# resemble-ai/chatterbox

Hardware: AMD Instinct MI355X
Metric: audio-sec/wall-sec (xRT) + p50 first-audio latency, Multilingual-V3 500M (higher is better)
Workload: dtype f32 (T3: exact fp32 MFMA; S3Gen: every fp32 operand = 2 fp16 planes h + l/2048 = 22 significand bits, 3 fp16 MFMA products per fp32 product in two fp32 accumulators: error at or below the exact-fp32 MFMA path; operand range checked on the device, bf16x6 repeat otherwise)

## Files before the change

### chatterbox_amd/_lib.py

```python
import ctypes
import os

import torch

_HERE = os.path.dirname(os.path.abspath(__file__))
LIB_PATH = os.environ.get("CBX_LIB_PATH") or os.path.join(_HERE, "libcbx_hip.so")

c_f = ctypes.c_void_p
c_int, c_long, c_float = ctypes.c_int, ctypes.c_long, ctypes.c_float


ABI_VERSION = 16


class GemmParams(ctypes.Structure):
    _fields_ = [
        ("A", c_f), ("W", c_f), ("C", c_f), ("bias", c_f), ("R", c_f), ("C2", c_f),
        ("act1_param", c_f), ("act2_param", c_f), ("lens", c_f),
        ("M", c_int), ("N", c_int), ("K", c_int),
        ("Cin", c_int), ("taps", c_int), ("dil", c_int), ("stride", c_int), ("pad_left", c_int), ("up", c_int),
        ("Tin", c_int), ("nz1", c_int), ("nz2", c_int), ("w_kn", c_int), ("swiglu", c_int),
        ("act1", c_int), ("act2", c_int),
        ("act1_slope", c_float), ("act2_slope", c_float), ("alpha", c_float), ("beta", c_float),
        ("lda", c_long), ("a_s1", c_long), ("a_s2", c_long),
# ... 118 lines not shown


class PrefillEmbed(ctypes.Structure):
    _fields_ = ([(k, c_int) for k in ("B", "cfg", "n_bos", "abs_pos", "S", "pos0", "dim")] + [("bos_id", ctypes.c_longlong), ("meta", c_f), ("ids", c_f), ("cond", c_f),
                                                                                               ("cond_stride", c_long)]
                + [(k, c_f) for k in ("text_emb", "text_pos", "speech_emb", "speech_pos", "x", "positions", "cache_rows", "last")])


class PlanesRef(ctypes.Structure):
    _fields_ = [("p", c_f), ("ld", c_long), ("lo", c_long)]


class CfmTBlock(ctypes.Structure):
    _fields_ = [(k, c_f) for k in ("n1_w", "n1_b", "n3_w", "n3_b", "bo", "b1", "b2")] + [(k, PlanesRef) for k in ("wqkv", "wo", "w1", "w2")]


class CfmStage(ctypes.Structure):
    _fields_ = ([(k, PlanesRef) for k in ("c1", "c2", "res", "tail")]
                + [(k, c_f) for k in ("c1_b", "n1_w", "n1_b", "c2_b", "n2_w", "n2_b", "res_b", "tail_b")]
                + [("cin", c_int), ("n_tb", c_int), ("tb", ctypes.POINTER(CfmTBlock))])


class CfmSolve(ctypes.Structure):
    _fields_ = ([(k, c_int) for k in ("n_stages", "rows", "B", "n_steps", "cfg", "fused_qkv", "fused_ln")]
                + [("T", c_long), ("cfg_rate", c_float), ("dt", ctypes.POINTER(c_float)), ("stages", ctypes.POINTER(CfmStage)),
                   ("fin_c", PlanesRef), ("fin_proj", PlanesRef)]
                + [(k, c_f) for k in ("fin_c_b", "fin_n_w", "fin_n_b", "fin_proj_b", "tbias", "lens", "xin")]
                + [("xinP", PlanesRef)] + [(k, c_f) for k in ("ra", "rb", "x", "v")]
                + [(k, PlanesRef) for k in ("aP", "hP", "qkP", "attP", "ffP", "xP", "yP", "catP", "vtP")]
                + [("gemm_tile", c_int), ("attn_version", c_int)])


class Conformer(ctypes.Structure):
    _fields_ = [(k, c_f) for k in ("ln_mha_w", "ln_mha_b", "w4", "b4", "wpos", "wo", "bo", "ln_ff_w", "ln_ff_b", "w1", "b1", "w2", "b2")]


class S3Encode(ctypes.Structure):
    _fields_ = ([(k, c_int) for k in ("B", "N", "n_enc", "n_up", "precision")] + [(k, c_f) for k in ("ids", "lens", "lens2")]
                + [(k, c_f) for k in ("emb", "e_w", "e_b", "e_lnw", "e_lnb", "u_w", "u_b", "u_lnw", "u_lnb", "pl1_w", "pl1_b", "pl2_w", "pl2_b", "up_w", "up_b",
                                      "after_w", "after_b", "proj_w", "proj_b")]
                + [("enc", ctypes.POINTER(Conformer)), ("up_enc", ctypes.POINTER(Conformer)), ("pe", c_f), ("pe2", c_f)]
                + [(k, c_f) for k in ("x0", "xa", "y1", "x2", "xu", "xb", "h", "q4", "pp", "att", "ff", "mu")])


class HiftF0(ctypes.Structure):
    _fields_ = [("B", c_int), ("T", c_long), ("mel", c_f), ("lens", c_f), ("f0_w", c_f * 5), ("f0_b", c_f * 5), ("cls_w", c_f), ("cls_b", c_f), ("src_w", c_f),
                ("src_b", c_float), ("phase", c_f), ("noise", c_f), ("buf0", c_f), ("buf1", c_f), ("f0", c_f), ("s", c_f), ("cum", c_f)]
# ... 112 lines not shown
    "cbx_hift_istft_rows_f32": ([c_f, c_f, c_f, c_int, c_long, c_long, c_float, c_int, c_f], c_int),
}


class CbxError(RuntimeError):
    pass


def _load():
    if not os.path.exists(LIB_PATH):
        raise ImportError(
            f"{LIB_PATH} is missing: build it with `python -m chatterbox_amd.build` (hipcc --offload-arch=gfx950). "
            "chatterbox_amd has no CPU / eager fallback.")
    lib = ctypes.CDLL(LIB_PATH)
    for name, (args, res) in _SIGS.items():
        try:
            fn = getattr(lib, name)
        except AttributeError as e:
            raise ImportError(f"libcbx_hip.so does not export {name} (stale build?)") from e
        fn.argtypes = args
        fn.restype = res
    if lib.cbx_abi_version() != ABI_VERSION:
        raise ImportError("libcbx_hip.so ABI version mismatch")
    return lib


lib = _load()


def check(rc, what=""):
    if rc != 0:
        raise CbxError(f"{what}: rc={rc}: {lib.cbx_last_error().decode(errors='replace')}")
```

### chatterbox_amd/csrc/attention_planes.hip

```cpp
#include <stdlib.h>
#include "cbx_common.h"

namespace {

typedef _Float16 f16x4 __attribute__((ext_vector_type(4)));
typedef _Float16 f16x8 __attribute__((ext_vector_type(8)));
typedef unsigned u32x4 __attribute__((ext_vector_type(4)));

__device__ __attribute__((aligned(16))) const unsigned cbx_attn_zero_page[4] = {0u, 0u, 0u, 0u};
typedef const __attribute__((address_space(1))) void* gptr_t;
typedef __attribute__((address_space(3))) void* lptr_t;

struct FlashPlArgs {
    const _Float16* q; const _Float16* k; const _Float16* vt; _Float16* o; const int* key_lens;
    int Tq, Tk;
    long q_sb, q_st, q_lo, k_sb, k_st, k_lo, vt_sb, vt_sd, vt_lo, o_sb, o_st, o_lo;
    float scale;
    int causal;
    int diag;
};

constexpr int PKT = 64;
constexpr int PL_TILE = 64 * 8 * 16;
constexpr int PL_STAGE = 4 * PL_TILE;
// ... 435 lines not shown
    const float l_tot = l_run + half_swap(l_run);
    const float inv = l_tot > 0.f ? 1.0f / l_tot : 0.f;
    if (qi < a.Tq) {
        _Float16* op = a.o + (long)z * a.o_sb + (long)qi * a.o_st + head * 64;
#pragma unroll
        for (int d = 0; d < 2; ++d)
#pragma unroll
            for (int g = 0; g < 4; ++g) {
                unsigned h0, l0, h1, l1;
                cbx_split2(ot[d][g * 4 + 0] * inv, ot[d][g * 4 + 1] * inv, h0, l0);
                cbx_split2(ot[d][g * 4 + 2] * inv, ot[d][g * 4 + 3] * inv, h1, l1);
                *reinterpret_cast<uint2*>(op + d * 32 + 8 * g + 4 * lh) = make_uint2(h0, h1);
                *reinterpret_cast<uint2*>(op + a.o_lo + d * 32 + 8 * g + 4 * lh) = make_uint2(l0, l1);
            }
    }
}

}

static int g_attn_pl_version = 0;
extern "C" int cbx_set_attn_planes_version(int v) {
    g_attn_pl_version = v;
    return 0;
}

extern "C" int cbx_flash_attn_planes_v(const void* q, const void* k, const void* vt, void* o, const int* key_lens, int nz1, int n_heads, int Tq,
                                       int Tk, long q_sb, long q_st, long q_lo, long k_sb, long k_st, long k_lo, long vt_sb, long vt_sd,
                                       long vt_lo, long o_sb, long o_st, long o_lo, float scale, int causal, int version, void* stream) {
    CBX_REQUIRE(version >= 0 && version <= 6, "flash_attn_planes: version %d (0 = default, 1 .. 6)", version);
    CBX_REQUIRE(q && k && vt && o, "flash_attn_planes: null operand");
    CBX_REQUIRE(Tq > 0 && Tk > 0 && nz1 > 0 && n_heads > 0, "flash_attn_planes: bad shape");
    CBX_REQUIRE((q_sb | q_st | q_lo | k_sb | k_st | k_lo | vt_sb | vt_sd | vt_lo) % 8 == 0 &&
                    (((uintptr_t)q | (uintptr_t)k | (uintptr_t)vt) & 15) == 0,
                "flash_attn_planes: q / k / v^T planes must be 16-byte aligned (strides and plane offsets multiples of 8 halves)");
    CBX_REQUIRE((o_sb | o_st | o_lo) % 4 == 0 && ((uintptr_t)o & 7) == 0, "flash_attn_planes: output planes must be 8-byte aligned");
    CBX_REQUIRE(vt_sd >= (Tk + 7) / 8 * 8, "flash_attn_planes: a V^T row must hold Tk rounded up to 8 keys (got stride %ld for Tk = %d)", vt_sd, Tk);
    FlashPlArgs a{reinterpret_cast<const _Float16*>(q), reinterpret_cast<const _Float16*>(k), reinterpret_cast<const _Float16*>(vt),
                  reinterpret_cast<_Float16*>(o), key_lens, Tq, Tk, q_sb, q_st, q_lo, k_sb, k_st, k_lo, vt_sb, vt_sd, vt_lo, o_sb, o_st, o_lo,
                  scale, causal, 0};
#ifdef CBX_DIAG
    a.diag = getenv("CBX_ATTN_DIAG") ? atoi(getenv("CBX_ATTN_DIAG")) : 0;
#endif
    const int forced = version ? version : g_attn_pl_version;
    const bool short_seq = forced == 0 && Tk <= 768 && (long)((Tq + 255) / 256) * n_heads * nz1 > 128;
    const int ver = forced ? forced : short_seq ? 1 : 4;
    const bool v2ok = !causal && k_st >= k_lo + 64 && (long)Tk * k_st * 2 < 0x7fffffffL && 64 * vt_sd * 2 < 0x7fffffffL && vt_sd >= vt_lo;
    if (ver >= 2 && v2ok) {
        constexpr int lds = 3 * PL_STAGE;
        static unsigned long long configured = 0;
        const int dev = cbx_device();
        if (!(configured >> dev & 1)) {
            hipError_t e1 = hipFuncSetAttribute(reinterpret_cast<const void*>(flash_attn_pl2_kernel<true>), hipFuncAttributeMaxDynamicSharedMemorySize, lds);
            hipError_t e2 = hipFuncSetAttribute(reinterpret_cast<const void*>(flash_attn_pl2_kernel<false>), hipFuncAttributeMaxDynamicSharedMemorySize, lds);
            hipError_t e3 = hipFuncSetAttribute(reinterpret_cast<const void*>((flash_attn_pl2_kernel<false, true>)), hipFuncAttributeMaxDynamicSharedMemorySize, lds);
            hipError_t e4 = hipFuncSetAttribute(reinterpret_cast<const void*>((flash_attn_pl2_kernel<false, true, 4>)), hipFuncAttributeMaxDynamicSharedMemorySize, lds);
            hipError_t e5 = hipFuncSetAttribute(reinterpret_cast<const void*>((flash_attn_pl2_kernel<false, true, 8, true>)), hipFuncAttributeMaxDynamicSharedMemorySize, lds);
            if (e4 == hipSuccess) e4 = e5;
            if (e3 == hipSuccess) e3 = e4;
            if (e2 == hipSuccess) e2 = e3;
            if (e1 != hipSuccess || e2 != hipSuccess) return cbx_set_error((int)(e1 != hipSuccess ? e1 : e2), "flash_attn_planes: cannot reserve %d B of LDS", lds);
            configured |= 1ull << dev;
        }
        dim3 grid2((Tq + 255) / 256, n_heads, nz1);
        const bool small_grid = forced == 0 && (long)grid2.x * n_heads * nz1 <= 128;
        if (ver == 5 || small_grid) hipLaunchKernelGGL((flash_attn_pl2_kernel<false, true, 4>), dim3((Tq + 127) / 128, n_heads, nz1), dim3(256), lds, (hipStream_t)stream, a);
        else if (ver == 6) hipLaunchKernelGGL((flash_attn_pl2_kernel<false, true, 8, true>), grid2, dim3(512), lds, (hipStream_t)stream, a);
        else if (ver == 3) hipLaunchKernelGGL(flash_attn_pl2_kernel<true>, grid2, dim3(512), lds, (hipStream_t)stream, a);
// ... 16 lines not shown
```

### chatterbox_amd/csrc/cbx_common.h

```cpp
#pragma once
#include <hip/hip_runtime.h>
#include <stdint.h>
#include <stdio.h>
#include "../../include/cbx.h"

typedef float f32x4 __attribute__((ext_vector_type(4)));
typedef float f32x16 __attribute__((ext_vector_type(16)));

#ifndef CBX_WT
#define CBX_WT 1
#endif
__device__ __forceinline__ void cbx_store_out(float* p, float v) {
#if CBX_WT == 1
    asm volatile("global_store_dword %0, %1, off sc1" ::"v"(p), "v"(v) : "memory");
#elif CBX_WT == 2
    asm volatile("global_store_dword %0, %1, off sc0 sc1" ::"v"(p), "v"(v) : "memory");
#elif CBX_WT == 3
    __builtin_nontemporal_store(v, p);
#else
    *p = v;
#endif
}
__device__ __forceinline__ void cbx_store_out4(float* p, f32x4 v) {
#if CBX_WT == 1
    asm volatile("global_store_dwordx4 %0, %1, off sc1\n\ts_nop 1" ::"v"(p), "v"(v) : "memory");
#elif CBX_WT == 2
    asm volatile("global_store_dwordx4 %0, %1, off sc0 sc1\n\ts_nop 1" ::"v"(p), "v"(v) : "memory");
#elif CBX_WT == 3
    __builtin_nontemporal_store(v, reinterpret_cast<f32x4*>(p));
#else
    *reinterpret_cast<f32x4*>(p) = v;
#endif
}
#define CBX_F16_LO_SCALE 2048.0f
int* cbx_range_flag();
int cbx_wave_frame_ms(const char* who, const float* wav, const long* row_off, const int* row_len, int R, long nf, double* ws, void* stream);
#ifdef __HIPCC__
__device__ __forceinline__ void cbx_amax4(float& amax, const f32x4 v) {
    asm("v_max3_f32 %0, |%1|, |%2|, %0" : "+v"(amax) : "v"(v[0]), "v"(v[1]));
    asm("v_max3_f32 %0, |%1|, |%2|, %0" : "+v"(amax) : "v"(v[2]), "v"(v[3]));
}
__device__ __forceinline__ void cbx_split2(float v0, float v1, unsigned& h, unsigned& l) {
    typedef _Float16 cbx_h2 __attribute__((ext_vector_type(2)));
    typedef float cbx_f2 __attribute__((ext_vector_type(2)));
    const cbx_f2 v = {v0, v1};
    h = __builtin_bit_cast(unsigned, __builtin_convertvector(v, cbx_h2));
    const cbx_f2 t = v * CBX_F16_LO_SCALE;
    asm("v_fma_mixlo_f16 %0, %1, %2, %3 op_sel:[0,0,0] op_sel_hi:[1,0,0]" : "=v"(l) : "v"(h), "s"(-CBX_F16_LO_SCALE), "v"(t[0]));
    asm("v_fma_mixhi_f16 %0, %1, %2, %3 op_sel:[1,0,0] op_sel_hi:[1,0,0]\n\ts_nop 1" : "+v"(l) : "v"(h), "s"(-CBX_F16_LO_SCALE), "v"(t[1]));
}
#endif

static inline int cbx_device() {
    int d = 0;
    return (hipGetDevice(&d) == hipSuccess && d >= 0 && d < 64) ? d : 0;
}

int cbx_stream_coresident(hipStream_t st);
// ... 274 lines not shown
```

### chatterbox_amd/csrc/stage_seams.hip

```cpp
#include "cbx_common.h"

namespace {

inline cbx_planes_t cols(const cbx_planes_t& P, long c0) { return cbx_planes_t{(char*)P.p + 2 * c0, P.ld, P.lo}; }
inline cbx_planes_t rows_from(const cbx_planes_t& P, long r0) { return cbx_planes_t{(char*)P.p + 2 * r0 * P.ld, P.ld, P.lo}; }

struct CfmCtx {
    const cbx_cfm_t* d;
    void* stream;
    int rows;
    long T, M;

    int conv(const cbx_planes_t& src, const cbx_planes_t& w, int N, int cin, int taps, float* out, const cbx_planes_t* outp, const float* bias,
             const float* R) const {
        cbx_gemm_pl_t g{};
        g.A = src.p, g.W = w.p, g.C = out, g.P = outp ? outp->p : nullptr, g.bias = bias, g.R = R;
        g.M = (int)T, g.N = N, g.K = taps * cin, g.Cin = cin, g.taps = taps, g.dil = 1, g.stride = 1, g.pad_left = taps - 1, g.Tin = (int)T, g.nz1 = rows;
        g.act = CBX_ACT_NONE, g.act_slope = 0.0f, g.alpha = 1.0f;
        g.lda = src.ld, g.a_lo = src.lo, g.a_s1 = T * src.ld;
        g.ldw = w.ld, g.w_lo = w.lo;
        if (out) g.ldc = N, g.c_s1 = T * N;
        if (R) g.ldr = N, g.r_s1 = T * N;
        if (outp) g.ldp = outp->ld, g.p_lo = outp->lo, g.p_s1 = T * outp->ld;
        g.tile = d->gemm_tile;
// ... 74 lines not shown
        return rc;
    }

    int estimator(const float* tbias) const {
        const int n = d->n_stages, n_mid = n - 2;
        const cbx_planes_t skip = cols(d->catP, 256), xh = d->catP;
        int rc;
        if ((rc = block(0, d->xinP, skip, tbias))) return rc;
        cbx_planes_t cur = n_mid == 0 ? xh : d->yP;
        if ((rc = conv(skip, d->stages[0].tail, 256, 256, 3, nullptr, &cur, d->stages[0].tail_b, nullptr))) return rc;
        for (int k = 1; k <= n_mid; ++k) {
            const cbx_planes_t nxt = k == n_mid ? xh : d->xP;
            if ((rc = block(k, cur, nxt, tbias))) return rc;
            cur = nxt;
        }
        if ((rc = block(n - 1, d->catP, d->xP, tbias))) return rc;
        if ((rc = conv(d->xP, d->stages[n - 1].tail, 256, 256, 3, nullptr, &d->yP, d->stages[n - 1].tail_b, nullptr))) return rc;
        if ((rc = conv(d->yP, d->fin_c, 256, 256, 3, d->ra, nullptr, d->fin_c_b, nullptr))) return rc;
        if ((rc = ln_planes(d->ra, d->aP, d->fin_n_w, d->fin_n_b, nullptr, CBX_ACT_MISH))) return rc;
        return conv(d->aP, d->fin_proj, 80, 256, 1, d->v, nullptr, d->fin_proj_b, nullptr);
    }
};

}

extern "C" int cbx_cfm_solve(const cbx_cfm_t* d, void* stream) {
    CBX_REQUIRE(d && d->stages && d->n_stages >= 2 && d->dt && d->tbias && d->xin && d->v && d->ra && d->rb && d->x, "cfm_solve: null descriptor field");
    CBX_REQUIRE(d->B >= 1 && d->T >= 1 && d->n_steps >= 1 && d->rows == (d->cfg ? 2 * d->B : d->B), "cfm_solve: rows must be B (no CFG) or 2 B (CFG)");
    CBX_REQUIRE(d->T % 2 == 0 && (long)d->rows * d->T > 32 && ((long)d->rows * d->T + 512) * 4096 < (1L << 31),
                "cfm_solve: the plane-format path needs an even T, rows * T > 32 and 31-bit operand offsets (rows * T = %ld)", (long)d->rows * d->T);
    for (int k = 0; k < d->n_stages; ++k) {
        const cbx_cfm_stage_t& s = d->stages[k];
        CBX_REQUIRE(s.n_tb >= 1 && s.tb && s.cin % 32 == 0, "cfm_solve: stage %d needs transformer blocks and cin %% 32 == 0", k);
        CBX_REQUIRE((s.tail.p != nullptr) == (k == 0 || k == d->n_stages - 1), "cfm_solve: the down and the up stage (only) end in a conv");
    }
    CfmCtx c{d, stream, d->rows, d->T, (long)d->rows * d->T};
    for (int k = 0; k < d->n_steps; ++k) {
        int rc;
        if (k && (rc = cbx_split_planes_f32(d->xin, d->xinP.p, c.M, 80, 320, d->xinP.ld, d->xinP.lo, stream))) return rc;
        if ((rc = c.estimator(d->tbias + (long)k * d->n_stages * 256))) return rc;
        if ((rc = cbx_cfm_euler_f32(d->xin, d->v, d->B, d->T, 80, 320, 80, d->T * 320, d->T * 80, d->dt[k], d->cfg_rate, d->cfg, stream))) return rc;
    }
    return 0;
}

namespace {

struct HiftCtx {
    const cbx_hift_t* d;
    void* stream;

    struct Conv {
        const float *x, *w, *bias, *res = nullptr, *p1 = nullptr, *p2 = nullptr;
        float *out, *out2 = nullptr;
        const int* lens = nullptr;
        long Tin, Tout, ldx, xs, ldo, os;
        int N, taps, cin, dil = 1, stride = 1, pad_left = 0, act1 = CBX_ACT_NONE, act2 = CBX_ACT_NONE;
        float slope1 = 0.0f, slope2 = 0.0f, alpha = 1.0f, beta = 0.0f;
    };
    int run(const Conv& c) const {
        cbx_gemm_t g{};
        g.A = c.x, g.W = c.w, g.C = c.out, g.bias = c.bias, g.R = c.res, g.C2 = c.out2, g.act1_param = c.p1, g.act2_param = c.p2, g.lens = c.lens;
        g.M = (int)c.Tout, g.N = c.N, g.K = c.taps * c.cin, g.Cin = c.cin, g.taps = c.taps, g.dil = c.dil, g.stride = c.stride, g.pad_left = c.pad_left;
        g.up = 1, g.Tin = (int)c.Tin, g.nz1 = d->B, g.nz2 = 1;
        g.act1 = c.act1, g.act2 = c.act2, g.act1_slope = c.slope1, g.act2_slope = c.slope2, g.alpha = c.alpha, g.beta = c.beta;
        g.lda = c.ldx, g.a_s1 = c.xs, g.ldw = (long)c.taps * c.cin, g.ldc = c.ldo, g.c_s1 = c.os;
        if (c.res) g.ldr = c.ldo, g.r_s1 = c.os;
// ... 195 lines not shown
```

### chatterbox_amd/engine.py

```python
import contextlib
import math
import os
import time
import warnings
from dataclasses import dataclass
from typing import Optional

import torch

from . import ops
from .hift import HiFTEngine
from .s3gen import FlowEngine
from .t3 import T3Engine, START_SPEECH, STOP_SPEECH

SPEECH_VOCAB = 6561
SAMPLES_PER_TOKEN = 960


RANGE_TRIPS = 0


def _range_checked(eng, run, check=True):
    out = run()
    if check and 16 in (eng.flow.precision, eng.hift.precision) and ops.range_flag_tripped():
# ... 439 lines not shown
        if d.join is not None:
            wavs = _joined_on_host(wavs.get("formatted", wavs["out"]), wavs["rec"], wavs["n"], d.fmt, wavs.get("pauses"), self._truncated(toks))
        self.last_timing["total_s"] = time.perf_counter() - t0
        return (wavs, st) if alignment is None else (wavs, st, alignment)

    @staticmethod
    def _truncated(toks):
        return [not bool((t == STOP_SPEECH).any()) for t in toks]
    @torch.inference_mode()
    def synthesize_pipelined(self, jobs, co_resident=True, host_threads=True, t3_in_flight=2, stream_priorities=(-1, 0), t3_pair=None, **kw):
        import threading
        jobs = [_checked_job(job) for job in jobs]
        for job in jobs:
            if "guard" in job:
                job["guard"] = self.t3.check_guard(job["guard"])
                if kw.get("ban_eos") or kw.get("ban_from", 0) > 0:
                    raise ValueError(GUARD_BANS)
        torch.cuda.set_device(self.dev)
        self._pipeline_streams(stream_priorities)
        t3_kw = {k: kw[k] for k in ("max_new_tokens", "temperature", "top_p", "min_p", "repetition_penalty", "cfg_weight", "ban_eos",
                                    "ban_from") if k in kw}
        job_kw = lambda job: dict(t3_kw, **{k: job[k] for k in ("temperature", "top_p", "min_p", "repetition_penalty", "cfg_weight", "guard") if k in job})
        self.co_resident(bool(co_resident))
        from ._lib import check, lib
        attr = bool(co_resident) and t3_in_flight < 2
        check(lib.cbx_set_stream_coresident(self._s_voc.cuda_stream, int(attr)), "cbx_set_stream_coresident")
        torch.cuda.synchronize()

        def enqueue_t3(job, box):
            try:
                torch.cuda.set_device(self.dev)
                with torch.inference_mode(), torch.cuda.stream(self._s_t3):
                    box["handle"] = self.t3.generate(job["t3_conds"], job["text_tokens"], async_mode=True, uniforms=job.get("uniforms"), seeds=job.get("seeds"), **job_kw(job))
            except BaseException as e:
                box["error"] = e

        def vocode_job(job, st):
            wavs, _ = self.vocode(st, job["gen_ref"], z=job.get("z"), phase=job.get("phase"), noise=job.get("noise"), generator=job.get("generator"), seeds=job.get("seeds"),
                                  speed=job.get("speed"), n_cfm_timesteps=kw.get("n_cfm_timesteps", 10), drop_last_token=kw.get("drop_last_token", True), sync=False,
                                  **({k: job[k] for k in ("join", "format", "loudness", "pauses", "pitch", "warp", "true_peak") if k in job}))
            if "warp" in job:
                job["_fit"] = self.last_fit
            return wavs

        def to_host(job, wavs, pinned):
            copy = (lambda w: torch.empty(w.shape, dtype=w.dtype, pin_memory=True).copy_(w, non_blocking=True)) if pinned else (lambda w: w.cpu())
# ... 12 lines not shown
            try:
                pending = None
                for k in range(len(jobs) + 1):
                    box = {}
                    if k < len(jobs):
                        t_start = time.perf_counter()
                        enqueue_t3(jobs[k], box)
                        if "error" in box:
                            raise box["error"]
                    if pending is not None:
                        job, st, t0, raw, rep = pending
                        with torch.cuda.stream(self._s_voc):
                            host = _range_checked(self, lambda: to_host(job, vocode_job(job, st), pinned=False))
                        self.last_guard, self.last_fit = rep, job.get("_fit")
                        yield result_of(job, host, raw), st, time.perf_counter() - t0
                    pending = None
                    if "handle" in box:
                        with torch.cuda.stream(self._s_t3):
                            raw = self.t3.collect(box["handle"])
                        pending = (jobs[k], _valid_tokens(raw), t_start, raw, self.t3.last_guard if "guard" in jobs[k] else None)
            finally:
                torch.cuda.synchronize()
                self.co_resident(False)
            return

        import queue
        n_t3 = max(1, min(3, int(t3_in_flight)))
        q, stop = queue.Queue(), threading.Event()
        n_slots = max(2, n_t3)
        slot_free = [threading.Semaphore(1) for _ in range(n_slots)]
        if t3_pair is None:
            t3_pair = bool(self.t3_pair) and os.environ.get("CBX_T3_PAIR", "1") != "0"
        units, k = [], 0
        while k < len(jobs):
            pair = None
            if t3_pair and k % 2 == 0 and k + 1 < len(jobs):
                pair = _paired_t3_call(jobs[k], jobs[k + 1], job_kw(jobs[k]), job_kw(jobs[k + 1]), int(kw.get("max_new_tokens", 1000)))
            units.append(([k, k + 1], pair) if pair is not None else ([k], None))
            k += len(units[-1][0])

        def worker():
            try:
                torch.cuda.set_device(self.dev)
                for u, (ks, pair) in enumerate(units):
                    slot_free[u % n_slots].acquire()
                    if stop.is_set():
# ... 44 lines not shown
                    self._s_voc.wait_event(ev)
                    toks_u = self.t3.collect(h)
                    rep = self.t3.last_guard if "guard" in jobs[ks[0]] else None
                slot_free[u % n_slots].release()
                lo = 0
                for k in ks:
                    job = jobs[k]
                    toks = toks_u[lo:lo + len(job["text_tokens"])]
                    lo += len(job["text_tokens"])
                    st = _valid_tokens(toks)
                    host, evv = start_voc(job, st, k % 2)
                    inflight.append((job, st, t0, host, evv, k % 2, toks, rep))
                    yield finish(*inflight.popleft())
            while inflight:
                yield finish(*inflight.popleft())
        finally:
            stop.set()
            for sem in slot_free:
                sem.release()
            th.join()
            ops.select_range_flag(self.dev, 0)
            torch.cuda.synchronize()
            self.co_resident(False)

    @torch.inference_mode()
    def synthesize_stream(self, text_tokens, t3_conds, gen_ref, *, first_chunk=25, chunk=50, chunk_growth=1.0, lookahead=3, fade=480, max_new_tokens=1000,
                          temperature=0.8, top_p=1.0, min_p=0.05, repetition_penalty=1.2, cfg_weight=0.5, uniforms=None, ban_eos=False,
                          ban_from=0, z=None, phase=None, noise=None, n_cfm_timesteps=10, drop_last_token=True, overlap=True, first_alone=True, run_ahead=2,
                          window=None, seeds=None, speed=None, format=None):
        t3_kw = dict(max_new_tokens=max_new_tokens, temperature=temperature, top_p=top_p, min_p=min_p, repetition_penalty=repetition_penalty,
                     cfg_weight=cfg_weight, uniforms=uniforms, ban_eos=ban_eos, ban_from=ban_from)

        yield from _synthesize_stream(self, text_tokens, t3_conds, gen_ref, n_budget=max_new_tokens, t3_kw=t3_kw, round_tokens=lambda toks, fin: _valid_tokens(toks), n_extra=0,
                                      first_chunk=first_chunk, chunk=chunk, chunk_growth=chunk_growth, lookahead=lookahead, fade=fade, z=z, phase=phase,
                                      noise=noise, n_cfm_timesteps=n_cfm_timesteps, drop_last_token=drop_last_token, overlap=overlap, first_alone=first_alone,
                                      run_ahead=run_ahead, window=window, seeds=seeds, speed=speed, format=format)


_T3_SAMPLING_DEFAULTS = dict(temperature=0.8, top_p=1.0, min_p=0.05, repetition_penalty=1.2, cfg_weight=0.5)


def _paired_t3_call(job_a, job_b, kw_a, kw_b, max_new_tokens):
    na, nb = len(job_a["text_tokens"]), len(job_b["text_tokens"])
    if 2 * (na + nb) > 32 or "guard" in kw_a or "guard" in kw_b:
        return None
    ua, ub = job_a.get("uniforms"), job_b.get("uniforms")
# ... 424 lines not shown
```

### chatterbox_amd/s3gen.py

```python
import math

import os

import torch

from . import ops, weights


def _dev(t, dev):
    return t.float().contiguous().to(dev)


class FlowEngine:
    @ops.on_device
    def __init__(self, sd, device="cuda", meanflow=False, precision=None):
        self.dev = dev = torch.device(device)
        self.meanflow = meanflow
        self.precision = int(os.environ.get("CBX_S3GEN_PRECISION", "16")) if precision is None else int(precision)
        ops.enable_range_flag(dev)
        d = lambda t: _dev(t, dev)
        self.emb = d(sd["flow.input_embedding.weight"])
        self.spk_w, self.spk_b = d(sd["flow.spk_embed_affine_layer.weight"]), d(sd["flow.spk_embed_affine_layer.bias"])
        self.proj_w, self.proj_b = d(sd["flow.encoder_proj.weight"]), d(sd["flow.encoder_proj.bias"])
        e = "flow.encoder."

        def embed(p):
            return dict(w=d(sd[p + "out.0.weight"]), b=d(sd[p + "out.0.bias"]), lnw=d(sd[p + "out.1.weight"]), lnb=d(sd[p + "out.1.bias"]))

        def conf(p):
            a = p + "self_attn."
            wq, bq = sd[a + "linear_q.weight"], sd[a + "linear_q.bias"]
            u, v = sd[a + "pos_bias_u"].reshape(-1), sd[a + "pos_bias_v"].reshape(-1)
            w4 = torch.cat([wq, wq, sd[a + "linear_k.weight"], sd[a + "linear_v.weight"]], 0)
# ... 45 lines not shown
            return s

        self.stages = [stage(q + "down_blocks.0.", True)]
        i = 0
        while f"{q}mid_blocks.{i}.0.mlp.1.weight" in sd:
            self.stages.append(stage(q + f"mid_blocks.{i}.", False))
            i += 1
        self.stages.append(stage(q + "up_blocks.0.", True))
        self.n_mid = i
        names = [q + "down_blocks.0."] + [q + f"mid_blocks.{k}." for k in range(i)] + [q + "up_blocks.0."]
        self.tmlp_w = d(torch.cat([sd[n + "0.mlp.1.weight"] for n in names], 0))
        self.tmlp_b = d(torch.cat([sd[n + "0.mlp.1.bias"] for n in names], 0))
        self.fin = dict(c=(d(weights.pack_conv(sd[q + "final_block.block.0.weight"])), d(sd[q + "final_block.block.0.bias"])),
                        n=(d(sd[q + "final_block.block.2.weight"]), d(sd[q + "final_block.block.2.bias"])),
                        proj=(d(weights.pack_conv(sd[q + "final_proj.weight"])), d(sd[q + "final_proj.bias"])))
        self._pe_cache, self._tb_cache = {}, {}
        self.use_planes = os.environ.get("CBX_PLANES", "1") != "0"
        self.fused_qkv = os.environ.get("CBX_FUSED_QKV", "1") != "0"
        self.fused_ln = int(os.environ.get("CBX_FUSED_LN", "0"))
        self._pw = None
        self.c_seam = True
        self._cfm_static = self._enc_static = None
        self.gemm_tile = self.attn_version = 0

    def co_resident(self, on):
        from ._lib import ATTN_PL_CORESIDENT, PL_TILE_CORESIDENT
        self.gemm_tile, self.attn_version = (PL_TILE_CORESIDENT, ATTN_PL_CORESIDENT) if on else (0, 0)

    def _rel_pos_table(self, T, dev=None, dm=512):
        if T not in self._pe_cache:
            pos = torch.arange(T - 1, -T, -1, dtype=torch.float32)[:, None]
            div = torch.exp(torch.arange(0, dm, 2, dtype=torch.float32) * -(math.log(10000.0) / dm))
            pe = torch.zeros(2 * T - 1, dm)
            pe[:, 0::2] = torch.sin(pos * div)
            pe[:, 1::2] = torch.cos(pos * div)
            if len(self._pe_cache) >= 16:
                self._pe_cache.pop(next(iter(self._pe_cache)))
            self._pe_cache[T] = pe.to(self.dev)
        return self._pe_cache[T]

    def _conformer(self, lw, x, B, T, pe, lens, ws):
        M = B * T
        h, q4 = ws["h"][:M], ws["q4"][:M]
        ops.layernorm(x, lw["ln_mha"][0], lw["ln_mha"][1], h, 1e-12)
        ops.linear(h, lw["w4"], q4, bias=lw["b4"])
        P = 2 * T - 1
        pp = ws["pp"][:P]
        ops.linear(pe, lw["wpos"], pp)
        q5 = q4.view(B, T, 4, 8, 64)
        att = ws["att"][:M]
# ... 254 lines not shown
            keep, stages = [], (CfmStage * len(self.stages))()
            for k, (sw, sp) in enumerate(zip(self.stages, pw["stages"])):
                tbs = (CfmTBlock * len(sw["tb"]))()
                for j, (tw, tp) in enumerate(zip(sw["tb"], sp["tb"])):
                    t = tbs[j]
                    t.n1_w, t.n1_b, t.n3_w, t.n3_b, t.bo, t.b1, t.b2 = (p(tw["n1"][0]), p(tw["n1"][1]), p(tw["n3"][0]), p(tw["n3"][1]), p(tw["bo"]),
                                                                        p(tw["b1"]), p(tw["b2"]))
                    t.wqkv, t.wo, t.w1, t.w2 = ref(tp["wqkv"]), ref(tp["wo"]), ref(tp["w1"]), ref(tp["w2"])
                st = stages[k]
                st.c1, st.c2, st.res = ref(sp["c1"]), ref(sp["c2"]), ref(sp["res"])
                st.c1_b, st.n1_w, st.n1_b, st.c2_b = p(sw["c1"][1]), p(sw["n1"][0]), p(sw["n1"][1]), p(sw["c2"][1])
                st.n2_w, st.n2_b, st.res_b = p(sw["n2"][0]), p(sw["n2"][1]), p(sw["res"][1])
                if "tail" in sw:
                    st.tail, st.tail_b = ref(sp["tail"]), p(sw["tail"][1])
                st.cin, st.n_tb, st.tb = int(sw["cin"]), len(sw["tb"]), tbs
                keep.append(tbs)
            d = CfmSolve()
            d.n_stages, d.stages = len(self.stages), stages
            d.fin_c, d.fin_proj = ref(pw["fin_c"]), ref(pw["fin_proj"])
            d.fin_c_b, d.fin_n_w, d.fin_n_b, d.fin_proj_b = p(self.fin["c"][1]), p(self.fin["n"][0]), p(self.fin["n"][1]), p(self.fin["proj"][1])
            self._cfm_static = (d, stages, keep)
        return self._cfm_static[0]

    def _cfm_solve_c(self, xin, xinP, lens_r, tb, t_span, ws, B, rows, T, n_steps, cfg, cfg_rate):
        import ctypes

        from ._lib import CfmSolve, PlanesRef, check, lib
        d = CfmSolve()
        ctypes.memmove(ctypes.byref(d), ctypes.byref(self._cfm_descriptor()), ctypes.sizeof(CfmSolve))
        ref = lambda P: PlanesRef(P.ptr, P.ld, P.lo)
        dt = (ctypes.c_float * n_steps)(*[float(t_span[k + 1] - t_span[k]) for k in range(n_steps)])
        assert tb.is_contiguous() and tb.shape == (n_steps, len(self.stages), 256) and lens_r.dtype == torch.int32 and lens_r.numel() == rows
        d.rows, d.B, d.n_steps, d.cfg, d.fused_qkv, d.fused_ln, d.T = rows, B, n_steps, int(cfg), int(self.fused_qkv), int(self.fused_ln), T
        d.cfg_rate, d.dt = cfg_rate, dt
        d.gemm_tile, d.attn_version = int(self.gemm_tile), int(self.attn_version)
        d.tbias, d.lens, d.xin, d.xinP = ops._p(tb), ops._p(lens_r), ops._p(xin), ref(xinP)
        d.ra, d.rb, d.x, d.v = ops._p(ws["ra"]), ops._p(ws["rb"]), ops._p(ws["x"]), ops._p(ws["v"])
        for k in ("aP", "hP", "qkP", "attP", "ffP", "xP", "yP", "catP", "vtP"):
            setattr(d, k, ref(ws[k]))
        check(lib.cbx_cfm_solve(ctypes.byref(d), ops._stream()), "cbx_cfm_solve")

    def _planes_ok(self, rows, T):
        return self.use_planes and ops.GEMM_PRECISION == 16 and rows * T > 32 and T % 2 == 0 and (rows * T + 512) * 4096 < 2 ** 31

    def _time_bias(self, t_vals, r_vals=None):
        dev = self.dev

        def tmlp(tv):
            half = 160
            fr = torch.exp(torch.arange(half).float() * -(math.log(10000) / (half - 1)))
            e = 1000.0 * tv[:, None] * fr[None]
            e = torch.cat([e.sin(), e.cos()], -1).to(dev)
            n = e.shape[0]
            h1, h2 = torch.empty(n, 1024, device=dev), torch.empty(n, 1024, device=dev)
            ops.linear(e, self.t1[0], h1, bias=self.t1[1], act=ops.SILU)
            ops.linear(h1, self.t2[0], h2, bias=self.t2[1])
            return h2
# ... 8 lines not shown
        ops.act(temb, m, ops.MISH)
        out = torch.empty(n, self.tmlp_w.shape[0], device=dev)
        ops.linear(m, self.tmlp_w, out, bias=self.tmlp_b)
        return out.view(n, -1, 256)

    @ops.on_device
    def cfm(self, mu, lens, spk, cond, z, n_steps=10, cfg_rate=0.7):
        dev, (B, T, _) = self.dev, mu.shape
        cfg = not self.meanflow
        rows = 2 * B if cfg else B
        f = lambda *s: torch.empty(*s, device=dev)
        planes = self._planes_ok(rows, T)
        if planes:
            M, Tp = rows * T, (T + 7) // 8 * 8
            PL = lambda C, **k: ops.Planes(M, C, dev, **k)
            ws = dict(ra=f(rows, T, 256), rb=f(rows, T, 256), x=f(rows, T, 256), v=f(rows, T, 80), aP=PL(256), hP=PL(256), qkP=PL(1024),
                      attP=PL(512), ffP=PL(1024), xP=PL(256), yP=PL(256), catP=PL(512),
                      vtP=ops.Planes(rows * 512, Tp, dev, zero=True))
        else:
            ws = dict(ra=f(rows, T, 256), rb=f(rows, T, 256), x=f(rows, T, 256), x2=f(rows, T, 256), y=f(rows, T, 256),
                      cat=f(rows, T, 512),
                      h=f(rows * T, 256), qkv=f(rows * T, 1536), att=f(rows * T, 512), ff=f(rows * T, 1024), v=f(rows, T, 80),
                      stats=f(rows * T, 2))
        xin = torch.zeros(rows, T, 320, device=dev)
        xin[:B, :, 0:80] = z
        xin[:B, :, 80:160] = mu
        xin[:B, :, 160:240] = spk[:, None, :]
        xin[:B, :, 240:320] = cond
        if cfg:
            xin[B:, :, 0:80] = z
        lens_r = torch.cat([lens, lens]).contiguous() if cfg else lens
        t_span = torch.linspace(0, 1, n_steps + 1)
        if not self.meanflow:
            t_span = 1 - torch.cos(t_span * 0.5 * math.pi)
        if n_steps not in self._tb_cache:
            self._tb_cache[n_steps] = self._time_bias(t_span[:-1], t_span[1:] if self.meanflow else None)
        tb = self._tb_cache[n_steps]
        if planes:
            xin2 = xin.view(rows * T, 320)
            xinP = ops.split_planes(xin2)
        if planes and self.c_seam and not ops.TIMER:
            self._cfm_solve_c(xin, xinP, lens_r, tb, t_span, ws, B, rows, T, n_steps, cfg, cfg_rate)
            return xin[:B, :, :80]
        for k in range(n_steps):
            if planes:
                if k:
                    ops.split_planes(xin2[:, :80], xinP.cols(0, 80))
                with ops.planes_geometry(self.gemm_tile, self.attn_version):
                    v = self._estimator_pl(xinP, rows, T, lens_r, tb[k], ws)
            else:
                v = self._estimator(xin, rows, T, lens_r, tb[k], ws)
            ops.cfm_euler(xin, v, B, T, 80, float(t_span[k + 1] - t_span[k]), cfg_rate, cfg=cfg)
        return xin[:B, :, :80]

    @ops.on_device
    @torch.inference_mode()
    def inference(self, tokens, token_lens, ref, z=None, n_steps=10, hold_back=None, generator=None, seeds=None):
        seeds = ops.request_seeds(seeds, tokens.shape[0], generator)
        with ops.gemm_precision(self.precision):
            return self._inference(tokens, token_lens, ref, z, n_steps, hold_back, generator, seeds)

    def _inference(self, tokens, token_lens, ref, z=None, n_steps=10, hold_back=None, generator=None, seeds=None):
        dev = self.dev
        B, N = tokens.shape
        refs = list(ref) if isinstance(ref, (list, tuple)) else [ref] * B
# ... 44 lines not shown
```

### include/cbx.h

```cpp
#ifndef CBX_H
#define CBX_H
#ifdef __cplusplus
extern "C" {
#endif

#define CBX_ABI_VERSION 16
#define CBX_EINVAL (-22)

enum { CBX_ACT_NONE = 0, CBX_ACT_SILU = 1, CBX_ACT_GELU_ERF = 2, CBX_ACT_GELU_TANH = 3, CBX_ACT_MISH = 4,
       CBX_ACT_LRELU = 5, CBX_ACT_ELU = 6, CBX_ACT_TANH = 7, CBX_ACT_SNAKE = 8, CBX_ACT_ABS = 9 };

int cbx_abi_version(void);
const char* cbx_last_error(void);

typedef struct cbx_gemm_t {
    const float* A; const float* W; float* C;
    const float* bias;
    const float* R;
    float* C2;
    const float* act1_param;
    const float* act2_param;
    const int* lens;
    int M, N, K;
    int Cin, taps, dil, stride, pad_left, up, Tin;
// ... 312 lines not shown
    long ld_logits;
    const cbx_sampler_t* sampler;
} cbx_gpt2_step_t;
int cbx_gpt2_decode_step(const cbx_gpt2_step_t* d, void* stream);
typedef struct cbx_gpt2_loop cbx_gpt2_loop_t;
int cbx_gpt2_loop_create(const cbx_gpt2_step_t* step, void* stream, cbx_gpt2_loop_t** out);
int cbx_gpt2_loop_run(cbx_gpt2_loop_t* h, int n_steps, int poll_every, void* stream, int* steps_run);
int cbx_gpt2_loop_destroy(cbx_gpt2_loop_t* h);

typedef struct cbx_planes_t { void* p; long ld, lo; } cbx_planes_t;

typedef struct cbx_cfm_tblock_t {
    const float *n1_w, *n1_b, *n3_w, *n3_b, *bo, *b1, *b2;
    cbx_planes_t wqkv, wo, w1, w2;
} cbx_cfm_tblock_t;
typedef struct cbx_cfm_stage_t {
    cbx_planes_t c1, c2, res, tail;
    const float *c1_b, *n1_w, *n1_b, *c2_b, *n2_w, *n2_b, *res_b, *tail_b;
    int cin, n_tb;
    const cbx_cfm_tblock_t* tb;
} cbx_cfm_stage_t;
typedef struct cbx_cfm_t {
    int n_stages, rows, B, n_steps, cfg, fused_qkv, fused_ln;
    long T;
    float cfg_rate;
    const float* dt;
    const cbx_cfm_stage_t* stages;
    cbx_planes_t fin_c, fin_proj;
    const float *fin_c_b, *fin_n_w, *fin_n_b, *fin_proj_b;
    const float* tbias;
    const int* lens;
    float* xin;
    cbx_planes_t xinP;
    float *ra, *rb, *x, *v;
    cbx_planes_t aP, hP, qkP, attP, ffP, xP, yP, catP;
    cbx_planes_t vtP;
    int gemm_tile, attn_version;
} cbx_cfm_t;
int cbx_cfm_solve(const cbx_cfm_t* d, void* stream);

typedef struct cbx_conformer_t {
    const float *ln_mha_w, *ln_mha_b, *w4, *b4, *wpos, *wo, *bo, *ln_ff_w, *ln_ff_b, *w1, *b1, *w2, *b2;
} cbx_conformer_t;
typedef struct cbx_s3enc_t {
    int B, N, n_enc, n_up, precision;
    const long long* ids;
// ... 140 lines not shown
```

Measured before the change: 231.0.

## Split CFM solve batch into two half-batch chains on forked streams

```diff
diff --git a/chatterbox_amd/_lib.py b/chatterbox_amd/_lib.py
--- a/chatterbox_amd/_lib.py
+++ b/chatterbox_amd/_lib.py
@@ -164,7 +164,7 @@
 
 
 class CfmSolve(ctypes.Structure):
-    _fields_ = ([(k, c_int) for k in ("n_stages", "rows", "B", "n_steps", "cfg", "fused_qkv", "fused_ln")]
+    _fields_ = ([(k, c_int) for k in ("n_stages", "rows", "B", "n_steps", "cfg", "fused_qkv", "fused_ln", "b_split")]
                 + [("T", c_long), ("cfg_rate", c_float), ("dt", ctypes.POINTER(c_float)), ("stages", ctypes.POINTER(CfmStage)),
                    ("fin_c", PlanesRef), ("fin_proj", PlanesRef)]
                 + [(k, c_f) for k in ("fin_c_b", "fin_n_w", "fin_n_b", "fin_proj_b", "tbias", "lens", "xin")]
@@ -323,6 +323,7 @@
         fn.restype = res
     if lib.cbx_abi_version() != ABI_VERSION:
         raise ImportError("libcbx_hip.so ABI version mismatch")
+    lib.cbx_cfm_two_chain_solves.argtypes, lib.cbx_cfm_two_chain_solves.restype = [], c_long
     return lib
 
 
diff --git a/chatterbox_amd/csrc/attention_planes.hip b/chatterbox_amd/csrc/attention_planes.hip
--- a/chatterbox_amd/csrc/attention_planes.hip
+++ b/chatterbox_amd/csrc/attention_planes.hip
@@ -481,6 +481,9 @@
 extern "C" int cbx_set_attn_planes_version(int v) {
     g_attn_pl_version = v;
     return 0;
+}
+bool cbx_attn_planes_short_seq(int Tq, int Tk, int n_heads, int nz1) {
+    return g_attn_pl_version == 0 && Tk <= 768 && (long)((Tq + 255) / 256) * n_heads * nz1 > 128;
 }
 
 extern "C" int cbx_flash_attn_planes_v(const void* q, const void* k, const void* vt, void* o, const int* key_lens, int nz1, int n_heads, int Tq,
@@ -501,7 +504,7 @@
     a.diag = getenv("CBX_ATTN_DIAG") ? atoi(getenv("CBX_ATTN_DIAG")) : 0;
 #endif
     const int forced = version ? version : g_attn_pl_version;
-    const bool short_seq = forced == 0 && Tk <= 768 && (long)((Tq + 255) / 256) * n_heads * nz1 > 128;
+    const bool short_seq = version == 0 && cbx_attn_planes_short_seq(Tq, Tk, n_heads, nz1);
     const int ver = forced ? forced : short_seq ? 1 : 4;
     const bool v2ok = !causal && k_st >= k_lo + 64 && (long)Tk * k_st * 2 < 0x7fffffffL && 64 * vt_sd * 2 < 0x7fffffffL && vt_sd >= vt_lo;
     if (ver >= 2 && v2ok) {
diff --git a/chatterbox_amd/csrc/cbx_common.h b/chatterbox_amd/csrc/cbx_common.h
--- a/chatterbox_amd/csrc/cbx_common.h
+++ b/chatterbox_amd/csrc/cbx_common.h
@@ -34,6 +34,7 @@
 }
 #define CBX_F16_LO_SCALE 2048.0f
 int* cbx_range_flag();
+bool cbx_attn_planes_short_seq(int Tq, int Tk, int n_heads, int nz1);
 int cbx_wave_frame_ms(const char* who, const float* wav, const long* row_off, const int* row_len, int R, long nf, double* ws, void* stream);
 #ifdef __HIPCC__
 __device__ __forceinline__ void cbx_amax4(float& amax, const f32x4 v) {
diff --git a/chatterbox_amd/csrc/stage_seams.hip b/chatterbox_amd/csrc/stage_seams.hip
--- a/chatterbox_amd/csrc/stage_seams.hip
+++ b/chatterbox_amd/csrc/stage_seams.hip
@@ -1,3 +1,5 @@
+#include <atomic>
+#include <mutex>
 #include "cbx_common.h"
 
 namespace {
@@ -120,6 +122,65 @@
     }
 };
 
+int cfm_step(const cbx_cfm_t& d, void* stream, int k0, int k1) {
+    CfmCtx c{&d, stream, d.rows, d.T, (long)d.rows * d.T};
+    for (int k = k0; k < k1; ++k) {
+        int rc;
+        if (k && (rc = cbx_split_planes_f32(d.xin, d.xinP.p, c.M, 80, 320, d.xinP.ld, d.xinP.lo, stream))) return rc;
+        if ((rc = c.estimator(d.tbias + (long)k * d.n_stages * 256))) return rc;
+        if ((rc = cbx_cfm_euler_f32(d.xin, d.v, d.B, d.T, 80, 320, 80, d.T * 320, d.T * 80, d.dt[k], d.cfg_rate, d.cfg, stream))) return rc;
+    }
+    return 0;
+}
+
+cbx_cfm_t cfm_half(const cbx_cfm_t& d, long r0, int B) {
+    cbx_cfm_t h = d;
+    const long m0 = r0 * d.T;
+    h.B = B, h.rows = d.cfg ? 2 * B : B, h.b_split = 0;
+    if (d.attn_version == 0 && cbx_attn_planes_short_seq((int)d.T, (int)d.T, 8, d.rows)) h.attn_version = 1;
+    if (h.lens) h.lens = d.lens + r0;
+    h.xin = d.xin + m0 * 320, h.ra = d.ra + m0 * 256, h.rb = d.rb + m0 * 256, h.x = d.x + m0 * 256, h.v = d.v + m0 * 80;
+    h.xinP = rows_from(d.xinP, m0), h.aP = rows_from(d.aP, m0), h.hP = rows_from(d.hP, m0), h.qkP = rows_from(d.qkP, m0), h.attP = rows_from(d.attP, m0);
+    h.ffP = rows_from(d.ffP, m0), h.xP = rows_from(d.xP, m0), h.yP = rows_from(d.yP, m0), h.catP = rows_from(d.catP, m0);
+    h.vtP = rows_from(d.vtP, r0 * 512);
+    return h;
+}
+
+std::atomic<long> g_two_chain_solves{0};
+
+#ifndef CBX_SIMT_EMU
+struct CfmSide {
+    int dev, prio;
+    hipStream_t st;
+    hipEvent_t fork, join;
+    std::mutex busy;
+};
+int cfm_side(hipStream_t caller, CfmSide** out) {
+    static std::mutex table_lock;
+    static std::vector<CfmSide*> table;
+    int prio = 0;
+    hipError_t e = hipStreamGetPriority(caller, &prio);
+    if (e != hipSuccess) return cbx_set_error((int)e, "cfm_solve: hipStreamGetPriority: %s", hipGetErrorString(e));
+    const int dev = cbx_device();
+    std::lock_guard<std::mutex> lock(table_lock);
+    for (CfmSide* s : table)
+        if (s->dev == dev && s->prio == prio) return *out = s, 0;
+    CfmSide* s = new CfmSide();
+    s->dev = dev, s->prio = prio, s->st = nullptr, s->fork = s->join = nullptr;
+    const char* what = "hipStreamCreateWithPriority";
+    if ((e = hipStreamCreateWithPriority(&s->st, hipStreamNonBlocking, prio)) == hipSuccess) what = "hipEventCreateWithFlags", e = hipEventCreateWithFlags(&s->fork, hipEventDisableTiming);
+    if (e == hipSuccess) e = hipEventCreateWithFlags(&s->join, hipEventDisableTiming);
+    if (e != hipSuccess) {
+        if (s->fork) (void)hipEventDestroy(s->fork);
+        if (s->st) (void)hipStreamDestroy(s->st);
+        delete s;
+        return cbx_set_error((int)e, "cfm_solve: %s: %s", what, hipGetErrorString(e));
+    }
+    table.push_back(s);
+    return *out = s, 0;
+}
+#endif
+
 }
 
 extern "C" int cbx_cfm_solve(const cbx_cfm_t* d, void* stream) {
@@ -132,15 +193,39 @@
         CBX_REQUIRE(s.n_tb >= 1 && s.tb && s.cin % 32 == 0, "cfm_solve: stage %d needs transformer blocks and cin %% 32 == 0", k);
         CBX_REQUIRE((s.tail.p != nullptr) == (k == 0 || k == d->n_stages - 1), "cfm_solve: the down and the up stage (only) end in a conv");
     }
-    CfmCtx c{d, stream, d->rows, d->T, (long)d->rows * d->T};
-    for (int k = 0; k < d->n_steps; ++k) {
-        int rc;
-        if (k && (rc = cbx_split_planes_f32(d->xin, d->xinP.p, c.M, 80, 320, d->xinP.ld, d->xinP.lo, stream))) return rc;
-        if ((rc = c.estimator(d->tbias + (long)k * d->n_stages * 256))) return rc;
-        if ((rc = cbx_cfm_euler_f32(d->xin, d->v, d->B, d->T, 80, 320, 80, d->T * 320, d->T * 80, d->dt[k], d->cfg_rate, d->cfg, stream))) return rc;
-    }
-    return 0;
-}
+    if (d->b_split == 0) return cfm_step(*d, stream, 0, d->n_steps);
+    CBX_REQUIRE(d->b_split > 0 && d->b_split < d->B, "cfm_solve: b_split %d does not split %d utterances", d->b_split, d->B);
+    const int per = d->cfg ? 2 : 1;
+    const cbx_cfm_t h0 = cfm_half(*d, 0, d->b_split), h1 = cfm_half(*d, (long)per * d->b_split, d->B - d->b_split);
+    CBX_REQUIRE((long)h0.rows * d->T >= 64 && (long)h1.rows * d->T >= 64, "cfm_solve: each half-batch needs rows * T >= 64 of its own");
+    int rc = 0;
+#ifndef CBX_SIMT_EMU
+    hipStreamCaptureStatus cap = hipStreamCaptureStatusNone;
+    hipError_t e = hipStreamIsCapturing((hipStream_t)stream, &cap);
+    if (e != hipSuccess) return cbx_set_error((int)e, "cfm_solve: hipStreamIsCapturing: %s", hipGetErrorString(e));
+    if (cap == hipStreamCaptureStatusNone) {
+        CfmSide* s = nullptr;
+        if ((rc = cfm_side((hipStream_t)stream, &s))) return rc;
+        std::lock_guard<std::mutex> lock(s->busy);
+        const int want = cbx_stream_coresident((hipStream_t)stream);
+        if (cbx_stream_coresident(s->st) != want && (rc = cbx_set_stream_coresident(s->st, want))) return rc;
+        const char* what = "hipEventRecord (fork)";
+        if ((e = hipEventRecord(s->fork, (hipStream_t)stream)) == hipSuccess) what = "hipStreamWaitEvent (fork)", e = hipStreamWaitEvent(s->st, s->fork, 0);
+        if (e != hipSuccess) return cbx_set_error((int)e, "cfm_solve: %s: %s", what, hipGetErrorString(e));
+        g_two_chain_solves.fetch_add(1);
+        for (int k = 0; !rc && k < d->n_steps; ++k)
+            if (!(rc = cfm_step(h0, stream, k, k + 1))) rc = cfm_step(h1, s->st, k, k + 1);
+        what = "hipEventRecord (join)";
+        if ((e = hipEventRecord(s->join, s->st)) == hipSuccess) what = "hipStreamWaitEvent (join)", e = hipStreamWaitEvent((hipStream_t)stream, s->join, 0);
+        if (!rc && e != hipSuccess) rc = cbx_set_error((int)e, "cfm_solve: %s: %s", what, hipGetErrorString(e));
+        return rc;
+    }
+#endif
+    if (!(rc = cfm_step(h0, stream, 0, d->n_steps))) rc = cfm_step(h1, stream, 0, d->n_steps);
+    return rc;
+}
+
+extern "C" long cbx_cfm_two_chain_solves(void) { return g_two_chain_solves.load(); }
 
 namespace {
 
diff --git a/chatterbox_amd/engine.py b/chatterbox_amd/engine.py
--- a/chatterbox_amd/engine.py
+++ b/chatterbox_amd/engine.py
@@ -485,6 +485,7 @@
                                     "ban_from") if k in kw}
         job_kw = lambda job: dict(t3_kw, **{k: job[k] for k in ("temperature", "top_p", "min_p", "repetition_penalty", "cfg_weight", "guard") if k in job})
         self.co_resident(bool(co_resident))
+        self.flow.two_chain_schedule = bool(co_resident) and bool(host_threads)
         from ._lib import check, lib
         attr = bool(co_resident) and t3_in_flight < 2
         check(lib.cbx_set_stream_coresident(self._s_voc.cuda_stream, int(attr)), "cbx_set_stream_coresident")
@@ -543,6 +544,7 @@
             finally:
                 torch.cuda.synchronize()
                 self.co_resident(False)
+                self.flow.two_chain_schedule = False
             return
 
         import queue
@@ -633,6 +635,7 @@
             ops.select_range_flag(self.dev, 0)
             torch.cuda.synchronize()
             self.co_resident(False)
+            self.flow.two_chain_schedule = False
 
     @torch.inference_mode()
     def synthesize_stream(self, text_tokens, t3_conds, gen_ref, *, first_chunk=25, chunk=50, chunk_growth=1.0, lookahead=3, fade=480, max_new_tokens=1000,
diff --git a/chatterbox_amd/s3gen.py b/chatterbox_amd/s3gen.py
--- a/chatterbox_amd/s3gen.py
+++ b/chatterbox_amd/s3gen.py
@@ -9,6 +9,28 @@
 
 def _dev(t, dev):
     return t.float().contiguous().to(dev)
+
+
+CFM_HALF_MIN_ROWS = 64
+
+
+def cfm_halves(B, cfg, chains):
+    per = 2 if cfg else 1
+    if chains != 2 or B < 2:
+        return [(0, B, 0)]
+    b0 = (B + 1) // 2
+    return [(0, b0, 0), (b0, B - b0, per * b0)]
+
+
+def cfm_row_order(B, cfg, chains):
+    out = []
+    for u0, n, _ in cfm_halves(B, cfg, chains):
+        out += [(u0 + i, False) for i in range(n)] + ([(u0 + i, True) for i in range(n)] if cfg else [])
+    return out
+
+
+def cfm_result_rows(B, cfg, chains):
+    return [r0 + i for _, n, r0 in cfm_halves(B, cfg, chains) for i in range(n)]
 
 
 class FlowEngine:
@@ -100,10 +122,18 @@
         self.c_seam = True
         self._cfm_static = self._enc_static = None
         self.gemm_tile = self.attn_version = 0
+        self.cfm_chains = int(os.environ.get("CBX_CFM_CHAINS", "0"))
+        self.two_chain_schedule = False
+        self.chains()
 
     def co_resident(self, on):
         from ._lib import ATTN_PL_CORESIDENT, PL_TILE_CORESIDENT
         self.gemm_tile, self.attn_version = (PL_TILE_CORESIDENT, ATTN_PL_CORESIDENT) if on else (0, 0)
+
+    def chains(self):
+        if self.cfm_chains not in (0, 1, 2):
+            raise ValueError(f"cfm_chains / CBX_CFM_CHAINS is 0 (automatic), 1 or 2, not {self.cfm_chains!r}")
+        return self.cfm_chains or (2 if self.two_chain_schedule else 1)
 
     def _rel_pos_table(self, T, dev=None, dm=512):
         if T not in self._pe_cache:
@@ -404,7 +434,7 @@
             self._cfm_static = (d, stages, keep)
         return self._cfm_static[0]
 
-    def _cfm_solve_c(self, xin, xinP, lens_r, tb, t_span, ws, B, rows, T, n_steps, cfg, cfg_rate):
+    def _cfm_solve_c(self, xin, xinP, lens_r, tb, t_span, ws, B, rows, T, n_steps, cfg, cfg_rate, b_split=0):
         import ctypes
 
         from ._lib import CfmSolve, PlanesRef, check, lib
@@ -415,6 +445,7 @@
         assert tb.is_contiguous() and tb.shape == (n_steps, len(self.stages), 256) and lens_r.dtype == torch.int32 and lens_r.numel() == rows
         d.rows, d.B, d.n_steps, d.cfg, d.fused_qkv, d.fused_ln, d.T = rows, B, n_steps, int(cfg), int(self.fused_qkv), int(self.fused_ln), T
         d.cfg_rate, d.dt = cfg_rate, dt
+        d.b_split = b_split
         d.gemm_tile, d.attn_version = int(self.gemm_tile), int(self.attn_version)
         d.tbias, d.lens, d.xin, d.xinP = ops._p(tb), ops._p(lens_r), ops._p(xin), ref(xinP)
         d.ra, d.rb, d.x, d.v = ops._p(ws["ra"]), ops._p(ws["rb"]), ops._p(ws["x"]), ops._p(ws["v"])
@@ -469,14 +500,23 @@
                       cat=f(rows, T, 512),
                       h=f(rows * T, 256), qkv=f(rows * T, 1536), att=f(rows * T, 512), ff=f(rows * T, 1024), v=f(rows, T, 80),
                       stats=f(rows * T, 2))
+        c_seam = planes and self.c_seam and not ops.TIMER
+        halves = cfm_halves(B, cfg, self.chains() if c_seam and not (dev.type == "cuda" and torch.cuda.is_current_stream_capturing()) else 1)
+        if min((2 if cfg else 1) * n * T for _, n, _ in halves) < CFM_HALF_MIN_ROWS:
+            halves = cfm_halves(B, cfg, 1)
         xin = torch.zeros(rows, T, 320, device=dev)
-        xin[:B, :, 0:80] = z
-        xin[:B, :, 80:160] = mu
-        xin[:B, :, 160:240] = spk[:, None, :]
-        xin[:B, :, 240:320] = cond
+        for u0, n, r0 in halves:
+            u = slice(u0, u0 + n)
+            xin[r0:r0 + n, :, 0:80] = z[u]
+            xin[r0:r0 + n, :, 80:160] = mu[u]
+            xin[r0:r0 + n, :, 160:240] = spk[u, None, :]
+            xin[r0:r0 + n, :, 240:320] = cond[u]
+            if cfg:
+                xin[r0 + n:r0 + 2 * n, :, 0:80] = z[u]
         if cfg:
-            xin[B:, :, 0:80] = z
-        lens_r = torch.cat([lens, lens]).contiguous() if cfg else lens
+            lens_r = torch.cat([lens[u0:u0 + n] for u0, n, _ in halves for _ in range(2)]).contiguous()
+        else:
+            lens_r = lens
         t_span = torch.linspace(0, 1, n_steps + 1)
         if not self.meanflow:
             t_span = 1 - torch.cos(t_span * 0.5 * math.pi)
@@ -486,8 +526,10 @@
         if planes:
             xin2 = xin.view(rows * T, 320)
             xinP = ops.split_planes(xin2)
-        if planes and self.c_seam and not ops.TIMER:
-            self._cfm_solve_c(xin, xinP, lens_r, tb, t_span, ws, B, rows, T, n_steps, cfg, cfg_rate)
+        if c_seam:
+            self._cfm_solve_c(xin, xinP, lens_r, tb, t_span, ws, B, rows, T, n_steps, cfg, cfg_rate, b_split=halves[0][1] if len(halves) == 2 else 0)
+            if len(halves) == 2 and cfg:
+                return torch.cat([xin[r0:r0 + n, :, :80] for _, n, r0 in halves])
             return xin[:B, :, :80]
         for k in range(n_steps):
             if planes:
diff --git a/include/cbx.h b/include/cbx.h
--- a/include/cbx.h
+++ b/include/cbx.h
@@ -358,6 +358,7 @@
 } cbx_cfm_stage_t;
 typedef struct cbx_cfm_t {
     int n_stages, rows, B, n_steps, cfg, fused_qkv, fused_ln;
+    int b_split;
     long T;
     float cfg_rate;
     const float* dt;
```

New measurement: 233.7 (median of 6 runs). 1.01x the previous value.
